# MatteoWohlrapp/mri-inr

Hardware: AMD Instinct MI355X
Metric: Mpixels/sec reconstructed (320x320 slice, hidden=256, 5 layers) (higher is better)
Workload: dtype f16x3

## Files before the change

mri_inr_amd/csrc/diagnostics.hip:

```cpp
#include <algorithm>
#include <vector>

#include "host_ctx.h"
#include "mfma_probe.hip.h"
#include "siren_trunk_f16x3n.hip.h"
#include "siren_trunk_f16x3w.hip.h"
#include "siren_trunk_f32.hip.h"
#include "trunk_instances.h"
#include "launch_dispatch.h"

namespace msiren {
MSIREN_F32_INSTANCES(MSIREN_EXTERN_TRUNK)
MSIREN_F16X3N_INSTANCES(MSIREN_EXTERN_TRUNK)
MSIREN_F16X3W_INSTANCES(MSIREN_EXTERN_TRUNK)
}

using namespace mh;

extern "C" {

int msiren_trunk_timeline(msiren_handle h, const float* mods_dev, int64_t B, float* out_dev, uint64_t* stamps_host) {
    int rc = check(h);
    if (rc) return rc;
    if (h->HP != 256 || h->cfg.activation != MSIREN_ACT_SINE || h->cfg.residual || h->H != 256)
// ... 4 lines not shown
    DevBuf st;
    if ((rc = ensure(h, st, (size_t)grid * 32 * sizeof(uint64_t)))) return rc;
    HIPCHK(hipMemsetAsync(st.p, 0, (size_t)grid * 32 * sizeof(uint64_t), h->sc[h->cur].s));
    msiren::TrunkParams p = make_trunk_params(h, Call{}, mods_dev, h->H, B, out_dev);
    p.stamps = (unsigned long long*)st.p;
    hipLaunchKernelGGL((msiren::siren_trunk_f32_kernel<256, 0, 0, 1>), dim3(grid), dim3(256), 256 * 256 + 256 * 16, h->sc[h->cur].s, p);
    HIPCHK(hipGetLastError());
    HIPCHK(hipMemcpyAsync(stamps_host, st.p, (size_t)grid * 32 * sizeof(uint64_t), hipMemcpyDeviceToHost, h->sc[h->cur].s));
    HIPCHK(hipStreamSynchronize(h->sc[h->cur].s));
    HIPCHK(hipFree(st.p));
    return 0;
}

int msiren_f16x3_timeline(msiren_handle h, const float* mods_dev, int64_t B, float* out_dev, uint64_t* stamps_host) {
    int rc = check(h);
    if (rc) return rc;
    if (!h->f16x3_ready || h->cfg.activation != MSIREN_ACT_SINE) return fail(MSIREN_E_INVALID, "f16x3 timeline: H=256 sine model required");
    msiren::TrunkF16Params p{};
    p.grid = h->d_grid; p.l0 = h->d_l0; p.s0t = h->d_s0t; p.wp = (const _Float16*)h->d_wp16n; p.bias = h->d_bias16;
    p.wout = h->d_wout16; p.mods = mods_dev; p.out = out_dev;
    for (int i = 0; i < 16; ++i) p.winv[i] = h->mscale16[i];
    p.bout = h->bout; p.cg0 = h->cg0; p.cg = h->cg; p.B = (int)B; p.P = h->P; p.L = h->L;
    p.units_per_patch = (h->P + 31) / 32;
    p.total_units = (int)(B * p.units_per_patch);
    const int grid = (int)std::min<int64_t>(h->num_cus, (p.total_units + 3) / 4);
    DevBuf st, q;
    if ((rc = ensure(h, st, (size_t)grid * 4 * 48 * sizeof(uint64_t))) || (rc = ensure(h, q, 256))) return rc;
    hipStream_t s = h->sc[h->cur].s;
    HIPCHK(hipMemsetAsync(st.p, 0, (size_t)grid * 4 * 48 * sizeof(uint64_t), s));
    p.pass_counter = (int*)q.p;
    HIPCHK(hipMemsetAsync(p.pass_counter, 0, 4, s));
    p.pass_base = 0;
    p.stamps = (unsigned long long*)st.p;
    const int lds = msiren::F16Lds<4>::total(h->L);
    {
        if (h->L != 5) return fail(MSIREN_E_INVALID, "f16x3 timeline: the stamped build is the num_layers = 5 instance");
        auto k = msiren::siren_trunk_f16x3n_kernel<0, 4, 5, 1>;
        HIPCHK(hipFuncSetAttribute((const void*)k, hipFuncAttributeMaxDynamicSharedMemorySize, lds));
        hipLaunchKernelGGL(k, dim3(grid), dim3(256), lds, s, p);
    }
    HIPCHK(hipGetLastError());
    HIPCHK(hipMemcpyAsync(stamps_host, st.p, (size_t)grid * 4 * 48 * sizeof(uint64_t), hipMemcpyDeviceToHost, s));
    HIPCHK(hipStreamSynchronize(s));
    HIPCHK(hipFree(st.p));
    HIPCHK(hipFree(q.p));
    return 0;
}

int msiren_f16x3w_timeline(msiren_handle h, const float* mods_dev, int64_t B, float* out_dev, uint64_t* stamps_host) {
    int rc = check(h);
    if (rc) return rc;
    if (!h->f16x3_ready || h->cfg.activation != MSIREN_ACT_SINE || h->L < msiren::WS_MIN_L || h->L > msiren::WS_MAX_L)
        return fail(MSIREN_E_INVALID, "f16x3w timeline: H=256 sine model with %d <= num_layers <= %d required", msiren::WS_MIN_L, msiren::WS_MAX_L);
    if (B <= 0 || !mods_dev || !out_dev || !stamps_host) return fail(MSIREN_E_INVALID, "bad arguments");
    msiren::TrunkWsParams p{};
    if (!h->d_dump) HIPCHK(hipMalloc((void**)&h->d_dump, 256 * sizeof(float)));
    p.dump = h->d_dump;
    p.s0t = h->d_s0t; p.wp = (const _Float16*)h->d_wp16n; p.bias = h->d_bias16; p.wout = h->d_wout16; p.mods = mods_dev; p.out = out_dev;
    for (int i = 0; i < 16; ++i) p.mscale[i] = h->mscale16[i];
    p.bout = h->bout; p.cg0 = h->cg0; p.cg = h->cg; p.B = (int)B; p.P = h->P; p.L = h->L;
    const int upp = (h->P + 31) / 32;
    p.units_per_patch = upp;
    p.total_units = (int)(B * upp);
    int lg = 0;
    while ((1 << lg) < upp) ++lg;
    p.div_k = 30 + lg;
// ... 68 lines not shown
```

mri_inr_amd/csrc/encoder_modulator_f16x3.hip.h:

```cpp
#pragma once
#include <hip/hip_runtime.h>

#include <type_traits>

#include "encoder_params.h"
#include "host_plan.h"

namespace msiren {

typedef _Float16 em_h8 __attribute__((ext_vector_type(8)));
typedef _Float16 em_h2 __attribute__((ext_vector_type(2)));
typedef float em_f4 __attribute__((ext_vector_type(4)));
typedef unsigned em_u4 __attribute__((ext_vector_type(4)));

constexpr int EM_ROWS = 16;
constexpr int EM_C3_KSTEPS = 64;
constexpr int EM_MAX_DEPTH = 16;
constexpr int EM_FC_KSTEPS = 4;

struct EmTailParams {
    const em_u4* wstream;
    const float* bias;
    const em_u4* feat;
    const float* feat_inv;
// ... 456 lines not shown
            for (int t = 0; t < 2; ++t) {
                const int pos = 16 * (2 * (wv >> 1) + t) + n, y = pos >> 3, x = pos & 7;
                const em_u4* src = a1img + ((2 * y + ky) * 17 + 2 * x + kx) * 4 + (q & 1);
                const em_u4 bh = src[0], bl = src[2];
                acc[t] = em_mfma(wa[s][1], bh, acc[t]);
                acc[t] = em_mfma(wa[s][0], bl, acc[t]);
                acc[t] = em_mfma(wa[s][0], bh, acc[t]);
            }
        }
        const float u = inv1 * p.c2_winv;
#pragma unroll
        for (int r = 0; r < 4; ++r) {
            o0[r] = leaky02(__builtin_fmaf(acc[0][r], u, b2[r]));
            o1[r] = leaky02(__builtin_fmaf(acc[1][r], u, b2[r]));
        }
    }
    float m = em_absmax8(o0, o1);
#pragma unroll
    for (int d = 1; d < 64; d <<= 1) m = __builtin_fmaxf(m, __shfl_xor(m, d));
    if (lane == 0) wmax[4 + wv] = m;
    __syncthreads();
    m = __builtin_fmaxf(__builtin_fmaxf(wmax[4], wmax[5]), __builtin_fmaxf(wmax[6], wmax[7]));
    float sc, inv;
    em_row_scale(m, sc, inv);
    em_u4 hi, lo;
    em_split8(o0 * sc, o1 * sc, hi, lo);
    const int row = blockIdx.x, ks = 16 * wv + (lane >> 2), qq = lane & 3;
    em_u4* dst = feat + ((size_t)(row >> 4) * EM_C3_KSTEPS + ks) * 128 + qq * 16 + (row & 15);
    dst[0] = hi;
    dst[64] = lo;
    if (tid == 0) feat_inv[row] = inv;
}

}
```

mri_inr_amd/csrc/host_ctx.h:

```cpp
#pragma once
#include <hip/hip_runtime.h>

#include <cstdint>
#include <map>
#include <string>
#include <vector>

#include "../../include/msiren.h"
#include "dispatch.h"
#include "encoder_params.h"
#include "pass_queue.h"

typedef struct ncclComm* ncclComm_t;

namespace mh {

int fail(int code, const char* fmt, ...) __attribute__((format(printf, 2, 3)));
const char* last_error();

#define HIPCHK(expr)                                                                              \
    do {                                                                                          \
        hipError_t e_ = (expr);                                                                   \
        if (e_ != hipSuccess)                                                                     \
            return ::mh::fail(MSIREN_E_HIP, "%s failed: %s (%s:%d)", #expr, hipGetErrorString(e_), __FILE__, __LINE__); \
    } while (0)

struct DevBuf {
    void* p = nullptr;
    size_t cap = 0;
};

}

struct msiren_ctx {
    msiren_config cfg{};
    int H = 0, HP = 0, L = 0, Z = 0, S = 0, P = 0, O = 0, I = 0;
    struct StreamCtx {
        hipStream_t s = nullptr;
        mh::DevBuf mods, modpad, latent, patches, keep, rec, queue, feat, plan;
        mh::DevBuf score;
        mh::DevBuf cscratch;
        mh::DevBuf coords, l0tab;
        mh::DevBuf ragged;
        struct Lattice {
            int out_stride = 0, tile = 0, pad = 0;
            float *coords = nullptr, *table = nullptr, *foldw = nullptr;
            std::vector<float> host;
        };
        std::vector<Lattice> lattices;
        hipEvent_t ev_join = nullptr;
        msiren::PassQueue pq;
    } sc[3];
    int cur = 0, nstreams = 1;
    msiren::DispatchHandle dh;
    const char* last_trunk = "";
    const char* last_prologue = "";
    struct { const void* k = nullptr; int bytes = 0; } lds_set[8];
    hipEvent_t ev0 = nullptr, ev1 = nullptr;
    std::map<std::string, std::vector<float>> tensors;
    std::map<std::string, size_t> expected;
    std::vector<float> grid_host;
    bool committed = false, have_modulator = false, have_encoder = false;
    float *d_grid = nullptr, *d_l0 = nullptr, *d_wp = nullptr, *d_bias = nullptr, *d_wout = nullptr;
    float *d_w0raw = nullptr, *d_b0raw = nullptr;
    float bout = 0.f, cg0 = 0.f, cg = 0.f;
    void* d_wp16n = nullptr;
    volatile int* status_host = nullptr;
    int* status_dev = nullptr;
    unsigned range_epoch = 0;
    int64_t range_events = 0;
    float* d_dump = nullptr;
    int trace_host = 0;
    float *d_bias16 = nullptr, *d_wout16 = nullptr, *d_s0t = nullptr;
// ... 167 lines not shown
```

mri_inr_amd/csrc/launch_dispatch.h:

```cpp
#pragma once
#include "host_ctx.h"

namespace mh {
msiren::TrunkParams make_trunk_params(msiren_ctx* h, const Call& c, const float* mods, int stride, int64_t B, float* out_dev);
}
```

mri_inr_amd/csrc/launch_dispatch.hip:

```cpp
#include <algorithm>
#include <cstdio>

#include "host_ctx.h"
#include "encoder_modulator.hip.h"
#include "encoder_modulator_f16x3.hip.h"
#include "siren_trunk_f16x3n.hip.h"
#include "siren_trunk_f16x3n_ragged.hip.h"
#include "siren_trunk_f16x3h.hip.h"
#include "siren_trunk_f16x3w.hip.h"
#include "siren_trunk_f32.hip.h"
#include "siren_trunk_f32_jet.hip.h"
#include "siren_trunk_f32_ragged.hip.h"
#include "siren_trunk_x1n.hip.h"
#include "siren_trunk_x1w.hip.h"
#include "tiling.hip.h"
#include "launch_dispatch.h"

namespace msiren {
MSIREN_TRUNK_INSTANCES(MSIREN_EXTERN_TRUNK)
MSIREN_F32_JET_INSTANCES(MSIREN_EXTERN_TRUNK)
MSIREN_F32_RAGGED_INSTANCES(MSIREN_EXTERN_TRUNK)
MSIREN_F32_JET_RAGGED_INSTANCES(MSIREN_EXTERN_TRUNK)
MSIREN_F16X3N_RAGGED_INSTANCES(MSIREN_EXTERN_TRUNK)
MSIREN_F32_RAGGED_COND_INSTANCES(MSIREN_EXTERN_TRUNK)
// ... 183 lines not shown
    p.bias = h->d_bias16;
    p.wout = h->d_wout16;
    p.mods = mods_dev;
    p.out = out_dev;
    for (int i = 0; i < 16; ++i) p.mscale[i] = h->mscale16[i];
    p.bout = h->bout;
    p.cg0 = h->cg0;
    p.cg = h->cg;
    p.B = (int)B;
    p.P = c.P(h);
    p.L = h->L;
    p.plan = c.plan;
    const int upp = (p.P + 31) / 32;
    const int64_t units = B * upp;
    if (units > 0x3fffffffLL) return fail(MSIREN_E_INVALID, "batch too large for one launch: B=%lld", (long long)B);
    p.units_per_patch = upp;
    p.unit_base = 0;
    p.total_units = (int)units;
    {
        int lg = 0;
        while ((1 << lg) < upp) ++lg;
        p.div_k = 30 + lg;
        p.div_m = (unsigned)(((1ULL << p.div_k) + (unsigned)upp - 1) / (unsigned)upp);
    }
    const int grid = (int)std::min<int64_t>(h->num_cus, (units + 1) / 2);
    const msiren::WsSchedule sch = msiren::ws_schedule(units, grid);
    int rc = queue_for_launch(h, c.stream, sch.npasses(), &p.pass_counter, &p.pass_base);
    if (rc) return rc;
    p.status = guard_word(h, t, p.pass_counter);
    p.status_val = (int)h->range_epoch;
    return queue_launched(h, c.stream, launch(h, c.stream, t.inst, grid, msiren::WsLds<4>::total(h->L), p, true));
}

static int launch_trunk_f16x3n(msiren_ctx* h, const Call& c, const msiren::TrunkPick& t, const float* mods_dev, int64_t B, float* out_dev) {
    msiren::TrunkF16Params p{};
    p.grid = c.cs.Q ? c.cs.coords : h->d_grid;
    p.l0 = h->d_l0;
    p.s0t = c.cs.Q ? c.cs.table : h->d_s0t;
    p.wp = (const _Float16*)h->d_wp16n;
    p.bias = h->d_bias16;
    p.wout = h->d_wout16;
    p.mods = mods_dev;
    p.out = out_dev;
    for (int i = 0; i < 16; ++i) p.winv[i] = h->mscale16[i];
    p.bout = h->bout;
    p.cg0 = h->cg0;
    p.cg = h->cg;
    p.B = (int)B;
    p.P = c.P(h);
    p.L = h->L;
    p.plan = c.plan;
    if (B * ((p.P + 31) / 32) > 0x3fffffffLL) return fail(MSIREN_E_INVALID, "batch too large for one launch: B=%lld", (long long)B);
    p.units_per_patch = t.half ? (p.P + 15) / 16 : (p.P + 31) / 32;
    p.unit_base = 0;
    p.total_units = (int)(B * p.units_per_patch);
    const int64_t passes = ((int64_t)p.total_units + 3) / 4;
    const int grid = (int)std::min<int64_t>(h->num_cus, passes);
    int rc = queue_for_launch(h, c.stream, passes, &p.pass_counter, &p.pass_base);
    if (rc) return rc;
    p.status = guard_word(h, t, p.pass_counter);
    p.status_val = (int)h->range_epoch;
    const int lds = t.ring == 4 ? msiren::F16Lds<4>::total(h->L) : msiren::F16Lds<3>::total(h->L);
    return queue_launched(h, c.stream, launch(h, c.stream, t.inst, grid, lds, p, true));
}

static int launch_trunk_x1(msiren_ctx* h, const Call& c, const msiren::TrunkPick& t, const float* mods_dev, int64_t B, float* out_dev) {
    const bool ws = msiren::kInstances[t.inst].family == Kernel::x1w;
    msiren::TrunkX1Params p{};
    p.s0t = c.cs.Q ? c.cs.table : h->d_s0t512;
    p.wp = (const unsigned short*)(ws ? h->d_wpx1w : h->d_wpx1n);
    p.bias32 = h->d_bias32x1;
    p.wout = (const _Float16*)h->d_woutx1;
    p.mods = mods_dev;
    p.out = out_dev;
    for (int i = 0; i < 64; ++i) p.winv[i] = h->winvx1[i];
    p.bout = h->bout;
    p.cg0 = h->cg0;
    p.cg = h->cg;
    p.B = (int)B;
    p.P = c.P(h);
    p.L = h->L;
    p.units_per_patch = (p.P + 31) / 32;
    const int64_t units = B * p.units_per_patch;
    if (units > 0x7fffffffLL) return fail(MSIREN_E_INVALID, "batch too large for one launch: B=%lld", (long long)B);
    p.total_units = (int)units;
    p.plan = c.plan;
    const int grid = t.balanced ? msiren::x1w_balanced_grid(units, h->num_cus) : (int)std::min<int64_t>(h->num_cus, (units + 3) / 4);
    int64_t npasses = (units + 3) / 4;
    if (ws) {
        const msiren::X1wSchedule sch = msiren::x1w_schedule(units, grid);
        npasses = (int64_t)sch.n4 + sch.n2;
    }
    int rc = queue_for_launch(h, c.stream, npasses, &p.pass_counter, &p.pass_base);
    if (rc) return rc;
// ... 627 lines not shown
```

mri_inr_amd/csrc/msiren.hip:

```cpp
#include <dlfcn.h>

#include <chrono>
#include <cstdarg>
#include <cstdio>
#include <cstdlib>
#include <cstring>

#include "host_ctx.h"
#include "host_buffers.h"
#include "host_plan.h"
#include "weights_blob.h"

namespace mh {

namespace {
thread_local std::string g_err;
}

int fail(int code, const char* fmt, ...) {
    char buf[1024];
    va_list ap;
    va_start(ap, fmt);
    vsnprintf(buf, sizeof buf, fmt, ap);
    va_end(ap);
// ... 167 lines not shown
        for (int i = 0; i < 16; ++i) h->status_host[i] = 0;
        e = hipHostGetDevicePointer((void**)&h->status_dev, (void*)h->status_host, 0);
    }

    if (e == hipSuccess) e = hipEventCreate(&h->ev0);
    if (e == hipSuccess) e = hipEventCreate(&h->ev1);
    if (e != hipSuccess) {
        msiren_destroy(h);
        return fail(MSIREN_E_HIP, "context creation failed: %s", hipGetErrorString(e));
    }
    *out = h;
    return 0;
}

int msiren_destroy(msiren_handle h) {
    if (!h) return 0;
    (void)hipSetDevice(h->cfg.device);
    for (auto& c : h->sc)
        if (c.s) (void)hipStreamSynchronize(c.s);
    if (h->comm) (void)comm_destroy(h);
    drop_lattices(h);
    if (h->status_host) (void)hipHostFree((void*)h->status_host);
    if (h->ws_comm.p) (void)hipFree(h->ws_comm.p);
    if (h->d_wp16n) (void)hipFree(h->d_wp16n);
    if (h->d_emw) (void)hipFree(h->d_emw);
    if (h->d_emc2) (void)hipFree(h->d_emc2);
    for (void* q : {h->d_woutx1, h->d_wpx1n, h->d_wpx1w, (void*)h->d_bias32x1})
        if (q) (void)hipFree(q);
    float* ptrs[] = {h->d_w0raw, h->d_b0raw, h->d_dump, h->d_s0t512, h->d_s0t, h->d_bias16, h->d_wout16, h->d_grid, h->d_l0, h->d_wp, h->d_bias, h->d_wout, h->d_modw, h->d_modw_rm, h->d_modb, h->d_encw, h->d_foldw, h->d_embias};
    for (float* p : ptrs)
        if (p) (void)hipFree(p);
    std::vector<DevBuf*> bufs = {&h->stage_in, &h->stage_out};
    for (auto& c : h->sc)
        for (DevBuf* b : {&c.cscratch, &c.mods, &c.modpad, &c.latent, &c.patches, &c.keep, &c.rec, &c.queue, &c.feat, &c.plan, &c.score, &c.coords, &c.l0tab, &c.ragged}) bufs.push_back(b);
    for (DevBuf* b : bufs)
        if (b->p) (void)hipFree(b->p);
    for (auto& pr : h->prof_events) {
        (void)hipEventDestroy(pr.a);
        (void)hipEventDestroy(pr.b);
    }
    for (auto& c : h->sc)
        if (c.ev_join) (void)hipEventDestroy(c.ev_join);
    if (h->ev0) (void)hipEventDestroy(h->ev0);
    if (h->ev1) (void)hipEventDestroy(h->ev1);
    for (auto& c : h->sc)
        if (c.s) (void)hipStreamDestroy(c.s);
    delete h;
    return 0;
}

int msiren_set_tensor(msiren_handle h, const char* name, const float* host_data, size_t n) {
    if (!h || !name || (!host_data && n)) return fail(MSIREN_E_INVALID, "null argument");
    auto it = h->expected.find(name);
    if (it == h->expected.end()) return fail(MSIREN_E_INVALID, "Unexpected key in state_dict: \"%s\"", name);
    if (it->second != n)
        return fail(MSIREN_E_SHAPE, "size mismatch for %s: got %zu elements, the configuration implies %zu", name, n, it->second);
    h->tensors[name].assign(host_data, host_data + n);
    h->committed = false;
    return 0;
}

int msiren_get_tensor(msiren_handle h, const char* name, float* host_out, size_t n) {
    if (!h || !name || (!host_out && n)) return fail(MSIREN_E_INVALID, "null argument");
    auto ex = h->expected.find(name);
    if (ex == h->expected.end()) return fail(MSIREN_E_INVALID, "Unexpected key in state_dict: \"%s\"", name);
    auto it = h->tensors.find(name);
    if (it == h->tensors.end()) return fail(MSIREN_E_STATE, "tensor %s has not been set", name);
// ... 505 lines not shown
```

mri_inr_amd/csrc/siren_trunk_f16x3h.hip.h:

```cpp
#pragma once
#include <hip/hip_runtime.h>

#include "siren_trunk_f16x3n.hip.h"

namespace msiren {

template <int ACT, int R, int LFIX = 0>
__global__ __launch_bounds__(256, 1) void siren_trunk_f16x3h_kernel(TrunkF16Params p) {
    using LY = F16Lds<R>;
    extern __shared__ __attribute__((aligned(16))) unsigned char smem[];
    const int tid = threadIdx.x;
    const int lane = tid & 63;
    const int wave = __builtin_amdgcn_readfirstlane(tid >> 6);
    const int q = lane >> 4;
    const int n16 = lane & 15;
    const int L = p.L;
    const int nchunks = (L - 1) * 8;

    const unsigned char* woutB = smem + LY::wout + q * 16;
    const unsigned char* zeroB = smem + LY::zero + q * 16;
    const unsigned char* biasB = smem + LY::bias + q * 16;
    float* modT = reinterpret_cast<float*>(smem + LY::mods(L)) + wave * (L * 256);
    const unsigned char* modB = reinterpret_cast<const unsigned char*>(modT) + q * 16;

    {
        f32x4* l0w = reinterpret_cast<f32x4*>(smem + LY::l0);
        float* wow = reinterpret_cast<float*>(smem + LY::wout);
        float* zw = reinterpret_cast<float*>(smem + LY::zero);
        float* bw = reinterpret_cast<float*>(smem + LY::bias);
        l0w[tid] = reinterpret_cast<const f32x4*>(p.l0)[tid];
        wow[tid] = p.wout[tid];
        zw[tid] = 0.f;
        for (int i = tid; i < (L - 1) * 256; i += 256) bw[i] = p.bias[i];
    }

    volatile int* qslot = reinterpret_cast<volatile int*>(smem + LY::queue(L));
    float* mscaleT = reinterpret_cast<float*>(smem + LY::winv(L));
    if (tid < 16) mscaleT[tid] = p.winv[tid];
    int cur_pass = (int)blockIdx.x;
    const unsigned char* wsrc = reinterpret_cast<const unsigned char*>(p.wp) + wave * 8192 + lane * 16 + 4096;
    int dma_id = 0, dma_buf = 0, rd_buf = 0;
    const unsigned char* dsrc_ = wsrc;
    unsigned char* ddst_ = smem + LY::ring + wave * 8192 + 4096;
    auto dma_begin = [&]() {
        dsrc_ = wsrc + (size_t)dma_id * F16_CHUNK_BYTES;
        ddst_ = smem + LY::ring + dma_buf * F16_CHUNK_BYTES + wave * 8192 + 4096;
        dma_id = dma_id + 1 == nchunks ? 0 : dma_id + 1;
        dma_buf = dma_buf + 1 == R ? 0 : dma_buf + 1;
    };
#define MSIREN_DMA_PIECE(I)                                                                               \
    __builtin_amdgcn_global_load_lds((const __attribute__((address_space(1))) void*)dsrc_,                \
                                     (__attribute__((address_space(3))) void*)ddst_, 16, (I) * 1024 - 4096, 0)
    auto dma_next = [&]() {
        dma_begin();
        MSIREN_DMA_PIECE(0);
        MSIREN_DMA_PIECE(1);
        MSIREN_DMA_PIECE(2);
        MSIREN_DMA_PIECE(3);
        MSIREN_DMA_PIECE(4);
        MSIREN_DMA_PIECE(5);
        MSIREN_DMA_PIECE(6);
        MSIREN_DMA_PIECE(7);
    };
    const int total_units = __builtin_amdgcn_readfirstlane(p.plan ? p.plan[1] : p.total_units);
    const unsigned npasses = (unsigned)(total_units + 3) >> 2;
    if ((unsigned)cur_pass >= npasses) return;
#pragma unroll
    for (int s = 0; s < R - 1; ++s) dma_next();

    h8 Xh[8], Xl[8], Yh[8], Yl[8];
    f32x4 acc[2][2];
    float part4[4] = {0.f, 0.f, 0.f, 0.f};

    fp16x2 eh[2][2], el[2][2];
    f32x4 tb_m[2], bia[2];
    auto tbl_load = [&](int sub, const unsigned char* ml, const unsigned char* wo, int t, bool withw) {
        const int fo = (32 * t + 16 * sub) * 4;
        tb_m[sub] = *reinterpret_cast<const f32x4*>(ml + fo);
        if (withw) tb_m[sub] *= *reinterpret_cast<const f32x4*>(wo + fo);
    };
    auto bias_load = [&](int sub, const unsigned char* bl, int t) {
        bia[sub] = *reinterpret_cast<const f32x4*>(bl + (32 * t + 16 * sub) * 4);
        asm("; bias fragment stays in arch VGPRs" : "+v"(bia[sub]));
    };
    auto epi_half = [&](const f32x4& a, float cgl, int sub, int hh, bool lastl, bool fresh = false, int chain = 0, bool ready = false) {
        float v[2];
        if (fresh) {
            v[0] = ready ? a[2 * hh] : activate<ACT>(a[2 * hh], cgl);
            v[1] = ready ? a[2 * hh + 1] : activate<ACT>(a[2 * hh + 1], cgl);
        } else if constexpr (ACT == 0) {
            asm volatile("v_sin_f32 %0, %1" : "=v"(v[0]) : "v"(a[2 * hh]));
            asm volatile("v_sin_f32 %0, %1" : "=v"(v[1]) : "v"(a[2 * hh + 1]));
        } else {
            float s0, s1, t0, t1;
            asm volatile("v_sin_f32 %0, %2\n\tv_mul_f32 %1, %3, %2" : "=&v"(s0), "=&v"(t0) : "v"(a[2 * hh]), "v"(cgl));
            asm volatile("v_sin_f32 %0, %2\n\tv_mul_f32 %1, %3, %2" : "=&v"(s1), "=&v"(t1) : "v"(a[2 * hh + 1]), "v"(cgl));
            v[0] = s0 * __builtin_amdgcn_exp2f(t0 * a[2 * hh]);
            v[1] = s1 * __builtin_amdgcn_exp2f(t1 * a[2 * hh + 1]);
        }
// ... 81 lines not shown
        const unsigned char* mlp_ = modB + (l_ - 1) * 1024;                                   \
        MSIREN_H16_TILE(INh, INl, OUTh, OUTl, 0, LASTF);                                        \
        MSIREN_H16_TILE(INh, INl, OUTh, OUTl, 1, LASTF);                                        \
        MSIREN_H16_TILE(INh, INl, OUTh, OUTl, 2, LASTF);                                        \
        MSIREN_H16_TILE(INh, INl, OUTh, OUTl, 3, LASTF);                                        \
        MSIREN_H16_TILE(INh, INl, OUTh, OUTl, 4, LASTF);                                        \
        MSIREN_H16_TILE(INh, INl, OUTh, OUTl, 5, LASTF);                                        \
        MSIREN_H16_TILE(INh, INl, OUTh, OUTl, 6, LASTF);                                        \
        MSIREN_H16_TILE(INh, INl, OUTh, OUTl, 7, LASTF);                                        \
    } while (0)

    asm volatile("s_waitcnt vmcnt(%0)" ::"n"((R - 2) * 8) : "memory");
    __syncthreads();
    bias_load(0, biasB, 0);
    bias_load(1, biasB, 0);
    {
        const h8* r0 = reinterpret_cast<const h8*>(smem + LY::ring) + lane;
        wf_[0][0] = r0[0 * 64];
        wf_[0][1] = r0[1 * 64];
        wf_[0][2] = r0[2 * 64];
        wf_[0][3] = r0[3 * 64];
    }

    for (int pass = 0; (unsigned)cur_pass < npasses; ++pass) {
        int unit = cur_pass * 4 + wave;
        const bool active = unit < total_units;
        unit = (active ? unit : total_units - 1) + p.unit_base;
        const int b = unit / p.units_per_patch;
        const int cu = unit - b * p.units_per_patch;
        int pc0 = cu * 16 + n16;
        const bool pv0 = active && pc0 < p.P;
        pc0 = pc0 < p.P ? pc0 : p.P - 1;

        int nxt = 0;
        if (tid == 0) nxt = (int)((unsigned)atomicAdd(p.pass_counter, 1) - p.pass_base) + (int)gridDim.x;
        bool bad_mod = false;
        for (int l = 0; l < L; ++l) {
            const f32x4 m = *reinterpret_cast<const f32x4*>(p.mods + ((size_t)l * p.B + b) * 256 + lane * 4);
            const f32x4 ms = m * mscaleT[l];
            bad_mod |= f16_out_of_range(ms);
            *reinterpret_cast<f32x4*>(modT + l * 256 + lane * 4) = ms;
        }
        if (bad_mod && p.status) *p.status = p.status_val;
        if (tid == 0) qslot[(pass + 1) & 1] = nxt;

        const f32x4* s0a = reinterpret_cast<const f32x4*>(p.s0t) + (size_t)q * p.P + pc0;
        f32x4 raw[7][2];
#pragma unroll
        for (int s = 0; s < 7; ++s)
#pragma unroll
            for (int sub = 0; sub < 2; ++sub) raw[s][sub] = s0a[(size_t)(8 * s + 4 * sub) * p.P];
#pragma unroll
        for (int s = 0; s < 7; ++s) {
            fp16x2 hh[2][2], ll[2][2];
#pragma unroll
            for (int sub = 0; sub < 2; ++sub) {
                const f32x4 m4 = *reinterpret_cast<const f32x4*>(modB + (32 * s + 16 * sub) * 4);
                const f32x4 a = raw[s][sub];
                split_products_pk(a[0], m4[0], a[1], m4[1], hh[sub][0], ll[sub][0]);
                split_products_pk(a[2], m4[2], a[3], m4[3], hh[sub][1], ll[sub][1]);
            }
            Xh[s] = to_acc_file(pack_h8(hh[0][0], hh[0][1], hh[1][0], hh[1][1]));
            Xl[s] = to_acc_file(pack_h8(ll[0][0], ll[0][1], ll[1][0], ll[1][1]));
        }
#pragma unroll
        for (int sub = 0; sub < 2; ++sub) acc[1][sub] = s0a[(size_t)(56 + 4 * sub) * p.P];
        tbl_load(0, modB, zeroB, 7, false);

        part4[0] = part4[1] = part4[2] = part4[3] = 0.f;
        if constexpr (LFIX == 5) {
            MSIREN_H16_LAYER(Xh, Xl, Yh, Yl, 1, false);
            MSIREN_H16_LAYER(Yh, Yl, Xh, Xl, 2, false);
            MSIREN_H16_LAYER(Xh, Xl, Yh, Yl, 3, false);
            MSIREN_H16_LAYER(Yh, Yl, Xh, Xl, 4, true);
        } else {
            for (int l = 1;;) {
                if (l == L - 1) {
                    MSIREN_H16_LAYER(Xh, Xl, Yh, Yl, l, true);
                    break;
                }
                MSIREN_H16_LAYER(Xh, Xl, Yh, Yl, l, false);
                ++l;
                if (l == L - 1) {
                    MSIREN_H16_LAYER(Yh, Yl, Xh, Xl, l, true);
                    break;
                }
                MSIREN_H16_LAYER(Yh, Yl, Xh, Xl, l, false);
                ++l;
            }
        }
        tbl_load(1, modB + (L - 1) * 1024, woutB, 7, true);
#pragma unroll
        for (int sub = 0; sub < 2; ++sub) {
            epi_half(acc[1][sub], p.cg, sub, 0, true, true, 3);
            epi_half(acc[1][sub], p.cg, sub, 1, true, true, 3);
        }
        const float sv = (sum_over_q(part4[0]) + sum_over_q(part4[1])) + (sum_over_q(part4[2]) + sum_over_q(part4[3]));
        if (q == 0 && pv0) p.out[(size_t)b * p.P + pc0] = sin_rev(sv + p.bout);
        cur_pass = __builtin_amdgcn_readfirstlane(qslot[(pass + 1) & 1]);
// ... 11 lines not shown
```

mri_inr_amd/csrc/siren_trunk_f16x3n.hip.h:

```cpp
#pragma once
#include <hip/hip_runtime.h>

#include "siren_trunk_f16_common.hip.h"

namespace msiren {

__device__ __forceinline__ void mfma_n16_first(f32x4& d, const h8& a, const h8& b, const f32x4& c) {
    d = __builtin_amdgcn_mfma_f32_16x16x32_f16(a, b, c, 0, 0, 0);
}
__device__ __forceinline__ void mfma_n16_acc(f32x4& d, const h8& a, const h8& b) {
    d = __builtin_amdgcn_mfma_f32_16x16x32_f16(a, b, d, 0, 0, 0);
}

__device__ __forceinline__ void split_products_pk(float a0, float m0, float a1, float m1, fp16x2& hi, fp16x2& lo) {
    unsigned h, l;
    asm("v_fma_mixlo_f16 %0, %1, %2, 0 op_sel_hi:[0,0,0]" : "=v"(h) : "v"(a0), "v"(m0));
    asm("v_fma_mixhi_f16 %0, %1, %2, 0 op_sel_hi:[0,0,0]" : "+v"(h) : "v"(a1), "v"(m1));
    asm("v_fma_mixlo_f16 %0, %1, %2, -%3 op_sel:[0,0,0] op_sel_hi:[0,0,1]" : "=v"(l) : "v"(a0), "v"(m0), "v"(h));
    asm("v_fma_mixhi_f16 %0, %1, %2, -%3 op_sel:[0,0,1] op_sel_hi:[0,0,1]" : "+v"(l) : "v"(a1), "v"(m1), "v"(h));
    hi = __builtin_bit_cast(fp16x2, h);
    lo = __builtin_bit_cast(fp16x2, l);
}

__device__ __forceinline__ float sum_over_q(float x) {
    float a = x, b = x;
    asm volatile("s_nop 1\n\tv_permlane16_swap_b32 %0, %1" : "+v"(a), "+v"(b));
    a += b;
    b = a;
    asm volatile("s_nop 1\n\tv_permlane32_swap_b32 %0, %1" : "+v"(a), "+v"(b));
    return a + b;
}


template <int ACT, int R, int LFIX = 0, int DBG = 0>
__global__ __launch_bounds__(256, 1) void siren_trunk_f16x3n_kernel(TrunkF16Params p) {
    using LY = F16Lds<R>;
    extern __shared__ __attribute__((aligned(16))) unsigned char smem[];
    const int tid = threadIdx.x;
    const int lane = tid & 63;
    const int wave = __builtin_amdgcn_readfirstlane(tid >> 6);
    const int q = lane >> 4;
    const int n16 = lane & 15;
    const int L = p.L;
    const int nchunks = (L - 1) * 8;

    const unsigned char* woutB = smem + LY::wout + q * 16;
    const unsigned char* zeroB = smem + LY::zero + q * 16;
    const unsigned char* biasB = smem + LY::bias + q * 16;
    float* modT = reinterpret_cast<float*>(smem + LY::mods(L)) + wave * (L * 256);
    const unsigned char* modB = reinterpret_cast<const unsigned char*>(modT) + q * 16;

    {
        f32x4* l0w = reinterpret_cast<f32x4*>(smem + LY::l0);
        float* wow = reinterpret_cast<float*>(smem + LY::wout);
        float* zw = reinterpret_cast<float*>(smem + LY::zero);
        float* bw = reinterpret_cast<float*>(smem + LY::bias);
        l0w[tid] = reinterpret_cast<const f32x4*>(p.l0)[tid];
        wow[tid] = p.wout[tid];
        zw[tid] = 0.f;
        for (int i = tid; i < (L - 1) * 256; i += 256) bw[i] = p.bias[i];
    }

    volatile int* qslot = reinterpret_cast<volatile int*>(smem + LY::queue(L));
    float* mscaleT = reinterpret_cast<float*>(smem + LY::winv(L));
    if (tid < 16) mscaleT[tid] = p.winv[tid];
    int cur_pass = (int)blockIdx.x;
    const unsigned char* wsrc = reinterpret_cast<const unsigned char*>(p.wp) + wave * 8192 + lane * 16 + 4096;
    int dma_id = 0, dma_buf = 0, rd_buf = 0;
    const unsigned char* dsrc_ = wsrc;
    unsigned char* ddst_ = smem + LY::ring + wave * 8192 + 4096;
    auto dma_begin = [&]() {
        dsrc_ = wsrc + (size_t)dma_id * F16_CHUNK_BYTES;
        ddst_ = smem + LY::ring + dma_buf * F16_CHUNK_BYTES + wave * 8192 + 4096;
        dma_id = dma_id + 1 == nchunks ? 0 : dma_id + 1;
        dma_buf = dma_buf + 1 == R ? 0 : dma_buf + 1;
    };
#define MSIREN_DMA_PIECE(I)                                                                               \
    __builtin_amdgcn_global_load_lds((const __attribute__((address_space(1))) void*)dsrc_,                \
                                     (__attribute__((address_space(3))) void*)ddst_, 16, (I) * 1024 - 4096, 0)
    auto dma_next = [&]() {
        dma_begin();
        MSIREN_DMA_PIECE(0);
        MSIREN_DMA_PIECE(1);
        MSIREN_DMA_PIECE(2);
        MSIREN_DMA_PIECE(3);
        MSIREN_DMA_PIECE(4);
        MSIREN_DMA_PIECE(5);
        MSIREN_DMA_PIECE(6);
        MSIREN_DMA_PIECE(7);
    };
    const int total_units = __builtin_amdgcn_readfirstlane(p.plan ? p.plan[1] : p.total_units);
    const unsigned npasses = (unsigned)(total_units + 3) >> 2;
    if ((unsigned)cur_pass >= npasses) return;
#pragma unroll
    for (int s = 0; s < R - 1; ++s) dma_next();

    h8 Xh[16], Xl[16], Yh[16], Yl[16];
    f32x4 acc[2][4];
    float part4[2][4] = {{0.f, 0.f, 0.f, 0.f}, {0.f, 0.f, 0.f, 0.f}};

    fp16x2 eh[4][2], el[4][2];
    f32x4 tb_m[2], bia[2];
    auto tbl_load = [&](int sub, const unsigned char* ml, const unsigned char* wo, int t, bool withw) {
        const int fo = (32 * t + 16 * sub) * 4;
        tb_m[sub] = *reinterpret_cast<const f32x4*>(ml + fo);
        if (withw) tb_m[sub] *= *reinterpret_cast<const f32x4*>(wo + fo);
    };
    auto bias_load = [&](int sub, const unsigned char* bl, int t) {
        bia[sub] = *reinterpret_cast<const f32x4*>(bl + (32 * t + 16 * sub) * 4);
        asm("; bias fragment stays in arch VGPRs" : "+v"(bia[sub]));
    };
    auto epi_half = [&](const f32x4& a, float cgl, int pt, int hh, bool lastl, bool fresh = false, int chain = 0, bool ready = false) {
        const int sub = pt & 1, g = pt >> 1;
        float v[2];
        if (fresh) {
            v[0] = ready ? a[2 * hh] : activate<ACT>(a[2 * hh], cgl);
            v[1] = ready ? a[2 * hh + 1] : activate<ACT>(a[2 * hh + 1], cgl);
        } else if constexpr (ACT == 0) {
            asm volatile("v_sin_f32 %0, %1" : "=v"(v[0]) : "v"(a[2 * hh]));
            asm volatile("v_sin_f32 %0, %1" : "=v"(v[1]) : "v"(a[2 * hh + 1]));
        } else {
            float s0, s1, t0, t1;
            asm volatile("v_sin_f32 %0, %2\n\tv_mul_f32 %1, %3, %2" : "=&v"(s0), "=&v"(t0) : "v"(a[2 * hh]), "v"(cgl));
            asm volatile("v_sin_f32 %0, %2\n\tv_mul_f32 %1, %3, %2" : "=&v"(s1), "=&v"(t1) : "v"(a[2 * hh + 1]), "v"(cgl));
            v[0] = s0 * __builtin_amdgcn_exp2f(t0 * a[2 * hh]);
            v[1] = s1 * __builtin_amdgcn_exp2f(t1 * a[2 * hh + 1]);
// ... 231 lines not shown

    asm volatile("s_waitcnt vmcnt(%0)" ::"n"((R - 2) * 8) : "memory");
    __syncthreads();
    bias_load(0, biasB, 0);
    bias_load(1, biasB, 0);
    {
        const h8* r0 = reinterpret_cast<const h8*>(smem + LY::ring) + lane;
        wf_[0][0] = r0[0 * 64];
        wf_[0][1] = r0[1 * 64];
        wf_[0][2] = r0[2 * 64];
        wf_[0][3] = r0[3 * 64];
    }

    for (int pass = 0; (unsigned)cur_pass < npasses; ++pass) {
        auto stamp = [&](int i) {
            if constexpr (DBG) {
                const unsigned long long t = i == 7 ? __builtin_amdgcn_s_memrealtime() : __builtin_amdgcn_s_memtime();
                if (tid == 0 && pass < 4) p.stamps[((size_t)blockIdx.x * 4 + pass) * 48 + i] = t;
            }
        };
        stamp(0);
        int dbg_tile = 0;
        (void)dbg_tile;
        int unit = cur_pass * 4 + wave;
        const bool active = unit < total_units;
        unit = (active ? unit : total_units - 1) + p.unit_base;
        const int b = unit / p.units_per_patch;
        const int cu = unit - b * p.units_per_patch;
        int pc0 = cu * 32 + n16, pc1 = cu * 32 + 16 + n16;
        const bool pv0 = active && pc0 < p.P, pv1 = active && pc1 < p.P;
        pc0 = pc0 < p.P ? pc0 : p.P - 1;
        pc1 = pc1 < p.P ? pc1 : p.P - 1;

        int nxt = 0;
        if (tid == 0) nxt = (int)((unsigned)atomicAdd(p.pass_counter, 1) - p.pass_base) + (int)gridDim.x;
        bool bad_mod = false;
        for (int l = 0; l < L; ++l) {
            const f32x4 m = *reinterpret_cast<const f32x4*>(p.mods + ((size_t)l * p.B + b) * 256 + lane * 4);
            const f32x4 ms = m * mscaleT[l];
            bad_mod |= f16_out_of_range(ms);
            *reinterpret_cast<f32x4*>(modT + l * 256 + lane * 4) = ms;
        }
        if (bad_mod && p.status) *p.status = p.status_val;
        if (tid == 0) qslot[(pass + 1) & 1] = nxt;

        const f32x4* s0a = reinterpret_cast<const f32x4*>(p.s0t) + (size_t)q * p.P + pc0;
        const f32x4* s0b = reinterpret_cast<const f32x4*>(p.s0t) + (size_t)q * p.P + pc1;
        f32x4 raw[14][2];
#pragma unroll
        for (int s = 0; s < 7; ++s)
#pragma unroll
            for (int sub = 0; sub < 2; ++sub) {
                raw[2 * s + 0][sub] = s0a[(size_t)(8 * s + 4 * sub) * p.P];
                raw[2 * s + 1][sub] = s0b[(size_t)(8 * s + 4 * sub) * p.P];
            }
#pragma unroll
        for (int s = 0; s < 7; ++s) {
            f32x4 m4[2];
#pragma unroll
            for (int sub = 0; sub < 2; ++sub) m4[sub] = *reinterpret_cast<const f32x4*>(modB + (32 * s + 16 * sub) * 4);
#pragma unroll
            for (int g = 0; g < 2; ++g) {
                fp16x2 hh[2][2], ll[2][2];
#pragma unroll
                for (int sub = 0; sub < 2; ++sub) {
                    const f32x4 a = raw[2 * s + g][sub];
                    split_products_pk(a[0], m4[sub][0], a[1], m4[sub][1], hh[sub][0], ll[sub][0]);
                    split_products_pk(a[2], m4[sub][2], a[3], m4[sub][3], hh[sub][1], ll[sub][1]);
                }
                Xh[2 * s + g] = to_acc_file(pack_h8(hh[0][0], hh[0][1], hh[1][0], hh[1][1]));
                Xl[2 * s + g] = to_acc_file(pack_h8(ll[0][0], ll[0][1], ll[1][0], ll[1][1]));
            }
        }
#pragma unroll
        for (int sub = 0; sub < 2; ++sub) {
            acc[1][0 + sub] = s0a[(size_t)(56 + 4 * sub) * p.P];
            acc[1][2 + sub] = s0b[(size_t)(56 + 4 * sub) * p.P];
        }
        tbl_load(0, modB, zeroB, 7, false);

#pragma unroll
        for (int c = 0; c < 4; ++c) part4[0][c] = part4[1][c] = 0.f;
        stamp(1);
        if constexpr (LFIX == 5) {
            MSIREN_N16_LAYER(Xh, Xl, Yh, Yl, 1, false);
            MSIREN_N16_LAYER(Yh, Yl, Xh, Xl, 2, false);
            MSIREN_N16_LAYER(Xh, Xl, Yh, Yl, 3, false);
            MSIREN_N16_LAYER(Yh, Yl, Xh, Xl, 4, true);
        } else {
            for (int l = 1;;) {
                if (l == L - 1) {
                    MSIREN_N16_LAYER(Xh, Xl, Yh, Yl, l, true);
                    break;
                }
                MSIREN_N16_LAYER(Xh, Xl, Yh, Yl, l, false);
                ++l;
                if (l == L - 1) {
                    MSIREN_N16_LAYER(Yh, Yl, Xh, Xl, l, true);
                    break;
                }
                MSIREN_N16_LAYER(Yh, Yl, Xh, Xl, l, false);
                ++l;
            }
        }
        stamp(2);
        tbl_load(1, modB + (L - 1) * 1024, woutB, 7, true);
#pragma unroll
        for (int pt = 0; pt < 4; ++pt) {
            epi_half(acc[1][pt], p.cg, pt, 0, true, true, 3);
            epi_half(acc[1][pt], p.cg, pt, 1, true, true, 3);
        }
// ... 23 lines not shown
```

Before: 385.9.

## Prescale modulations in a staging kernel and DMA them directly into LDS

Adds a small pre-pass kernel that multiplies the modulations by their per-layer f16 scale and checks their range once per batch row. For the L=5 f16x3n path, and unconditionally in the f16x3h kernel, the trunk then streams mods, l0, bias and wout into LDS with global_load_lds_dwordx4 instead of loading through registers, scaling and storing them. The s0 tail loads move earlier behind an explicit waitcnt, and the pass-counter atomic result is published later to overlap its latency. This removes per-pass VALU work and register round-trips, at the cost of an extra kernel launch plus a round trip of the mods through a global staging buffer.

```diff
diff --git a/mri_inr_amd/csrc/diagnostics.hip b/mri_inr_amd/csrc/diagnostics.hip
--- a/mri_inr_amd/csrc/diagnostics.hip
+++ b/mri_inr_amd/csrc/diagnostics.hip
@@ -60,6 +60,7 @@
     HIPCHK(hipMemsetAsync(p.pass_counter, 0, 4, s));
     p.pass_base = 0;
     p.stamps = (unsigned long long*)st.p;
+    if ((rc = stage_mods_f16x3(h, h->cur, mods_dev, B, nullptr, nullptr, 0, &p.mods))) return rc;
     const int lds = msiren::F16Lds<4>::total(h->L);
     {
         if (h->L != 5) return fail(MSIREN_E_INVALID, "f16x3 timeline: the stamped build is the num_layers = 5 instance");
diff --git a/mri_inr_amd/csrc/encoder_modulator_f16x3.hip.h b/mri_inr_amd/csrc/encoder_modulator_f16x3.hip.h
--- a/mri_inr_amd/csrc/encoder_modulator_f16x3.hip.h
+++ b/mri_inr_amd/csrc/encoder_modulator_f16x3.hip.h
@@ -512,4 +512,31 @@
     if (tid == 0) feat_inv[row] = inv;
 }
 
-}
+struct StageModsParams {
+    const float* mods;
+    float* staged;
+    float scale[16];
+    int B, L;
+    const int* count;
+    int* status;
+    int status_val;
+};
+
+template <int ROWS_PER_BLOCK = 4>
+__global__ __launch_bounds__(256) void stage_mods_f16x3_kernel(StageModsParams p) {
+    const int nrows = p.count ? *p.count : p.B;
+    const int64_t row = (int64_t)blockIdx.x * ROWS_PER_BLOCK + (threadIdx.x >> 6);
+    if (row >= nrows) return;
+    const int lane = threadIdx.x & 63;
+    bool bad = false;
+    for (int l = 0; l < p.L; ++l) {
+        const size_t at = ((size_t)l * p.B + row) * 256 + lane * 4;
+        const em_f4 ms = *reinterpret_cast<const em_f4*>(p.mods + at) * p.scale[l];
+#pragma unroll
+        for (int r = 0; r < 4; ++r) bad |= !(__builtin_fabsf(ms[r]) <= 65504.f);
+        *reinterpret_cast<em_f4*>(p.staged + at) = ms;
+    }
+    if (bad && p.status) *p.status = p.status_val;
+}
+
+}
diff --git a/mri_inr_amd/csrc/host_ctx.h b/mri_inr_amd/csrc/host_ctx.h
--- a/mri_inr_amd/csrc/host_ctx.h
+++ b/mri_inr_amd/csrc/host_ctx.h
@@ -39,6 +39,7 @@
         hipStream_t s = nullptr;
         mh::DevBuf mods, modpad, latent, patches, keep, rec, queue, feat, plan;
         mh::DevBuf score;
+        mh::DevBuf smods;
         mh::DevBuf cscratch;
         mh::DevBuf coords, l0tab;
         mh::DevBuf ragged;
diff --git a/mri_inr_amd/csrc/launch_dispatch.h b/mri_inr_amd/csrc/launch_dispatch.h
--- a/mri_inr_amd/csrc/launch_dispatch.h
+++ b/mri_inr_amd/csrc/launch_dispatch.h
@@ -3,4 +3,5 @@
 
 namespace mh {
 msiren::TrunkParams make_trunk_params(msiren_ctx* h, const Call& c, const float* mods, int stride, int64_t B, float* out_dev);
+int stage_mods_f16x3(msiren_ctx* h, int s, const float* mods_dev, int64_t B, const int* count, int* status, int status_val, const float** staged);
 }
diff --git a/mri_inr_amd/csrc/launch_dispatch.hip b/mri_inr_amd/csrc/launch_dispatch.hip
--- a/mri_inr_amd/csrc/launch_dispatch.hip
+++ b/mri_inr_amd/csrc/launch_dispatch.hip
@@ -239,6 +239,25 @@
     return queue_launched(h, c.stream, launch(h, c.stream, t.inst, grid, msiren::WsLds<4>::total(h->L), p, true));
 }
 
+int stage_mods_f16x3(msiren_ctx* h, int s, const float* mods_dev, int64_t B, const int* count, int* status, int status_val, const float** staged) {
+    auto& sc = h->sc[s];
+    int rc = ensure(h, sc.smods, (size_t)h->L * B * 256 * sizeof(float));
+    if (rc) return rc;
+    msiren::StageModsParams sp{};
+    sp.mods = mods_dev;
+    sp.staged = (float*)sc.smods.p;
+    for (int i = 0; i < 16; ++i) sp.scale[i] = h->mscale16[i];
+    sp.B = (int)B;
+    sp.L = h->L;
+    sp.count = count;
+    sp.status = status;
+    sp.status_val = status_val;
+    hipLaunchKernelGGL(msiren::stage_mods_f16x3_kernel<4>, dim3((unsigned)((B + 3) / 4)), dim3(256), 0, sc.s, sp);
+    HIPCHK(hipGetLastError());
+    *staged = sp.staged;
+    return 0;
+}
+
 static int launch_trunk_f16x3n(msiren_ctx* h, const Call& c, const msiren::TrunkPick& t, const float* mods_dev, int64_t B, float* out_dev) {
     msiren::TrunkF16Params p{};
     p.grid = c.cs.Q ? c.cs.coords : h->d_grid;
@@ -267,6 +286,7 @@
     if (rc) return rc;
     p.status = guard_word(h, t, p.pass_counter);
     p.status_val = (int)h->range_epoch;
+    if (h->L == 5 && (rc = stage_mods_f16x3(h, c.stream, mods_dev, B, c.plan, p.status, p.status_val, &p.mods))) return queue_launched(h, c.stream, rc);
     const int lds = t.ring == 4 ? msiren::F16Lds<4>::total(h->L) : msiren::F16Lds<3>::total(h->L);
     return queue_launched(h, c.stream, launch(h, c.stream, t.inst, grid, lds, p, true));
 }
diff --git a/mri_inr_amd/csrc/msiren.hip b/mri_inr_amd/csrc/msiren.hip
--- a/mri_inr_amd/csrc/msiren.hip
+++ b/mri_inr_amd/csrc/msiren.hip
@@ -223,7 +223,7 @@
         if (p) (void)hipFree(p);
     std::vector<DevBuf*> bufs = {&h->stage_in, &h->stage_out};
     for (auto& c : h->sc)
-        for (DevBuf* b : {&c.cscratch, &c.mods, &c.modpad, &c.latent, &c.patches, &c.keep, &c.rec, &c.queue, &c.feat, &c.plan, &c.score, &c.coords, &c.l0tab, &c.ragged}) bufs.push_back(b);
+        for (DevBuf* b : {&c.cscratch, &c.smods, &c.mods, &c.modpad, &c.latent, &c.patches, &c.keep, &c.rec, &c.queue, &c.feat, &c.plan, &c.score, &c.coords, &c.l0tab, &c.ragged}) bufs.push_back(b);
     for (DevBuf* b : bufs)
         if (b->p) (void)hipFree(b->p);
     for (auto& pr : h->prof_events) {
diff --git a/mri_inr_amd/csrc/siren_trunk_f16x3h.hip.h b/mri_inr_amd/csrc/siren_trunk_f16x3h.hip.h
--- a/mri_inr_amd/csrc/siren_trunk_f16x3h.hip.h
+++ b/mri_inr_amd/csrc/siren_trunk_f16x3h.hip.h
@@ -23,20 +23,7 @@
     float* modT = reinterpret_cast<float*>(smem + LY::mods(L)) + wave * (L * 256);
     const unsigned char* modB = reinterpret_cast<const unsigned char*>(modT) + q * 16;
 
-    {
-        f32x4* l0w = reinterpret_cast<f32x4*>(smem + LY::l0);
-        float* wow = reinterpret_cast<float*>(smem + LY::wout);
-        float* zw = reinterpret_cast<float*>(smem + LY::zero);
-        float* bw = reinterpret_cast<float*>(smem + LY::bias);
-        l0w[tid] = reinterpret_cast<const f32x4*>(p.l0)[tid];
-        wow[tid] = p.wout[tid];
-        zw[tid] = 0.f;
-        for (int i = tid; i < (L - 1) * 256; i += 256) bw[i] = p.bias[i];
-    }
-
-    volatile int* qslot = reinterpret_cast<volatile int*>(smem + LY::queue(L));
-    float* mscaleT = reinterpret_cast<float*>(smem + LY::winv(L));
-    if (tid < 16) mscaleT[tid] = p.winv[tid];
+    volatile __attribute__((address_space(3))) int* qslot = (volatile __attribute__((address_space(3))) int*)(smem + LY::queue(L));
     int cur_pass = (int)blockIdx.x;
     const unsigned char* wsrc = reinterpret_cast<const unsigned char*>(p.wp) + wave * 8192 + lane * 16 + 4096;
     int dma_id = 0, dma_buf = 0, rd_buf = 0;
@@ -65,6 +52,13 @@
     const int total_units = __builtin_amdgcn_readfirstlane(p.plan ? p.plan[1] : p.total_units);
     const unsigned npasses = (unsigned)(total_units + 3) >> 2;
     if ((unsigned)cur_pass >= npasses) return;
+    {
+        copy_1kb_to_lds(reinterpret_cast<const unsigned char*>(p.l0) + wave * 1024 + lane * 16, lds_address(smem + LY::l0) + wave * 1024);
+        for (int l = wave; l < L - 1; l += 4)
+            copy_1kb_to_lds(reinterpret_cast<const unsigned char*>(p.bias) + l * 1024 + lane * 16, lds_address(smem + LY::bias) + l * 1024);
+        if (wave == 0) copy_1kb_to_lds(reinterpret_cast<const unsigned char*>(p.wout) + lane * 16, lds_address(smem + LY::wout));
+        reinterpret_cast<float*>(smem + LY::zero)[tid] = 0.f;
+    }
 #pragma unroll
     for (int s = 0; s < R - 1; ++s) dma_next();
 
@@ -212,17 +206,19 @@
         const bool pv0 = active && pc0 < p.P;
         pc0 = pc0 < p.P ? pc0 : p.P - 1;
 
-        int nxt = 0;
-        if (tid == 0) nxt = (int)((unsigned)atomicAdd(p.pass_counter, 1) - p.pass_base) + (int)gridDim.x;
-        bool bad_mod = false;
-        for (int l = 0; l < L; ++l) {
-            const f32x4 m = *reinterpret_cast<const f32x4*>(p.mods + ((size_t)l * p.B + b) * 256 + lane * 4);
-            const f32x4 ms = m * mscaleT[l];
-            bad_mod |= f16_out_of_range(ms);
-            *reinterpret_cast<f32x4*>(modT + l * 256 + lane * 4) = ms;
-        }
-        if (bad_mod && p.status) *p.status = p.status_val;
-        if (tid == 0) qslot[(pass + 1) & 1] = nxt;
+        unsigned got = 0;
+        if (tid == 0) {
+            __attribute__((address_space(1))) int* pc = (__attribute__((address_space(1))) int*)p.pass_counter;
+            asm("" : "+v"(pc));
+            got = (unsigned)__hip_atomic_fetch_add(pc, 1, __ATOMIC_RELAXED, __HIP_MEMORY_SCOPE_AGENT);
+        }
+        {
+            const unsigned char* msrc = reinterpret_cast<const unsigned char*>(p.mods + (size_t)b * 256) + lane * 16;
+            const size_t mstep = (size_t)p.B * 1024;
+            const unsigned mdst = lds_address(modT);
+            for (int l = 0; l < L; ++l) copy_1kb_to_lds(msrc + l * mstep, mdst + l * 1024);
+        }
+        __builtin_amdgcn_sched_barrier(0);
 
         const f32x4* s0a = reinterpret_cast<const f32x4*>(p.s0t) + (size_t)q * p.P + pc0;
         f32x4 raw[7][2];
@@ -230,6 +226,10 @@
         for (int s = 0; s < 7; ++s)
 #pragma unroll
             for (int sub = 0; sub < 2; ++sub) raw[s][sub] = s0a[(size_t)(8 * s + 4 * sub) * p.P];
+#pragma unroll
+        for (int sub = 0; sub < 2; ++sub) acc[1][sub] = s0a[(size_t)(56 + 4 * sub) * p.P];
+        asm volatile("" ::: "memory");
+        __builtin_amdgcn_s_waitcnt(0x4F70);
 #pragma unroll
         for (int s = 0; s < 7; ++s) {
             fp16x2 hh[2][2], ll[2][2];
@@ -243,8 +243,7 @@
             Xh[s] = to_acc_file(pack_h8(hh[0][0], hh[0][1], hh[1][0], hh[1][1]));
             Xl[s] = to_acc_file(pack_h8(ll[0][0], ll[0][1], ll[1][0], ll[1][1]));
         }
-#pragma unroll
-        for (int sub = 0; sub < 2; ++sub) acc[1][sub] = s0a[(size_t)(56 + 4 * sub) * p.P];
+        if (tid == 0) qslot[(pass + 1) & 1] = (int)(got - p.pass_base) + (int)gridDim.x;
         tbl_load(0, modB, zeroB, 7, false);
 
         part4[0] = part4[1] = part4[2] = part4[3] = 0.f;
diff --git a/mri_inr_amd/csrc/siren_trunk_f16x3n.hip.h b/mri_inr_amd/csrc/siren_trunk_f16x3n.hip.h
--- a/mri_inr_amd/csrc/siren_trunk_f16x3n.hip.h
+++ b/mri_inr_amd/csrc/siren_trunk_f16x3n.hip.h
@@ -30,6 +30,11 @@
     asm volatile("s_nop 1\n\tv_permlane32_swap_b32 %0, %1" : "+v"(a), "+v"(b));
     return a + b;
 }
+
+__device__ __forceinline__ void copy_1kb_to_lds(const void* src, unsigned lds) {
+    asm volatile("s_mov_b32 m0, %1\n\ts_nop 0\n\tglobal_load_lds_dwordx4 %0, off" ::"v"(src), "s"(lds) : "memory", "m0");
+}
+__device__ __forceinline__ unsigned lds_address(const void* p) { return (unsigned)(size_t)(const __attribute__((address_space(3))) void*)p; }
 
 
 template <int ACT, int R, int LFIX = 0, int DBG = 0>
@@ -43,6 +48,9 @@
     const int n16 = lane & 15;
     const int L = p.L;
     const int nchunks = (L - 1) * 8;
+    if constexpr (DBG) {
+        if (tid == 0) p.stamps[(size_t)blockIdx.x * 4 * 48 + 3] = __builtin_amdgcn_s_memtime();
+    }
 
     const unsigned char* woutB = smem + LY::wout + q * 16;
     const unsigned char* zeroB = smem + LY::zero + q * 16;
@@ -50,20 +58,7 @@
     float* modT = reinterpret_cast<float*>(smem + LY::mods(L)) + wave * (L * 256);
     const unsigned char* modB = reinterpret_cast<const unsigned char*>(modT) + q * 16;
 
-    {
-        f32x4* l0w = reinterpret_cast<f32x4*>(smem + LY::l0);
-        float* wow = reinterpret_cast<float*>(smem + LY::wout);
-        float* zw = reinterpret_cast<float*>(smem + LY::zero);
-        float* bw = reinterpret_cast<float*>(smem + LY::bias);
-        l0w[tid] = reinterpret_cast<const f32x4*>(p.l0)[tid];
-        wow[tid] = p.wout[tid];
-        zw[tid] = 0.f;
-        for (int i = tid; i < (L - 1) * 256; i += 256) bw[i] = p.bias[i];
-    }
-
-    volatile int* qslot = reinterpret_cast<volatile int*>(smem + LY::queue(L));
-    float* mscaleT = reinterpret_cast<float*>(smem + LY::winv(L));
-    if (tid < 16) mscaleT[tid] = p.winv[tid];
+    volatile __attribute__((address_space(3))) int* qslot = (volatile __attribute__((address_space(3))) int*)(smem + LY::queue(L));
     int cur_pass = (int)blockIdx.x;
     const unsigned char* wsrc = reinterpret_cast<const unsigned char*>(p.wp) + wave * 8192 + lane * 16 + 4096;
     int dma_id = 0, dma_buf = 0, rd_buf = 0;
@@ -92,6 +87,23 @@
     const int total_units = __builtin_amdgcn_readfirstlane(p.plan ? p.plan[1] : p.total_units);
     const unsigned npasses = (unsigned)(total_units + 3) >> 2;
     if ((unsigned)cur_pass >= npasses) return;
+    if constexpr (LFIX != 0) {
+        copy_1kb_to_lds(reinterpret_cast<const unsigned char*>(p.l0) + wave * 1024 + lane * 16, lds_address(smem + LY::l0) + wave * 1024);
+        for (int l = wave; l < L - 1; l += 4)
+            copy_1kb_to_lds(reinterpret_cast<const unsigned char*>(p.bias) + l * 1024 + lane * 16, lds_address(smem + LY::bias) + l * 1024);
+        if (wave == 0) copy_1kb_to_lds(reinterpret_cast<const unsigned char*>(p.wout) + lane * 16, lds_address(smem + LY::wout));
+        reinterpret_cast<float*>(smem + LY::zero)[tid] = 0.f;
+    } else {
+        f32x4* l0w = reinterpret_cast<f32x4*>(smem + LY::l0);
+        float* wow = reinterpret_cast<float*>(smem + LY::wout);
+        float* zw = reinterpret_cast<float*>(smem + LY::zero);
+        float* bw = reinterpret_cast<float*>(smem + LY::bias);
+        l0w[tid] = reinterpret_cast<const f32x4*>(p.l0)[tid];
+        wow[tid] = p.wout[tid];
+        zw[tid] = 0.f;
+        for (int i = tid; i < (L - 1) * 256; i += 256) bw[i] = p.bias[i];
+        if (tid < 16) reinterpret_cast<float*>(smem + LY::winv(L))[tid] = p.winv[tid];
+    }
 #pragma unroll
     for (int s = 0; s < R - 1; ++s) dma_next();
 
@@ -389,21 +401,33 @@
         pc0 = pc0 < p.P ? pc0 : p.P - 1;
         pc1 = pc1 < p.P ? pc1 : p.P - 1;
 
-        int nxt = 0;
-        if (tid == 0) nxt = (int)((unsigned)atomicAdd(p.pass_counter, 1) - p.pass_base) + (int)gridDim.x;
-        bool bad_mod = false;
-        for (int l = 0; l < L; ++l) {
-            const f32x4 m = *reinterpret_cast<const f32x4*>(p.mods + ((size_t)l * p.B + b) * 256 + lane * 4);
-            const f32x4 ms = m * mscaleT[l];
-            bad_mod |= f16_out_of_range(ms);
-            *reinterpret_cast<f32x4*>(modT + l * 256 + lane * 4) = ms;
-        }
-        if (bad_mod && p.status) *p.status = p.status_val;
-        if (tid == 0) qslot[(pass + 1) & 1] = nxt;
+        unsigned got = 0;
+        if (tid == 0) {
+            __attribute__((address_space(1))) int* pc = (__attribute__((address_space(1))) int*)p.pass_counter;
+            asm("" : "+v"(pc));
+            got = (unsigned)__hip_atomic_fetch_add(pc, 1, __ATOMIC_RELAXED, __HIP_MEMORY_SCOPE_AGENT);
+        }
+        if constexpr (LFIX != 0) {
+            const unsigned char* msrc = reinterpret_cast<const unsigned char*>(p.mods + (size_t)b * 256) + lane * 16;
+            const size_t mstep = (size_t)p.B * 1024;
+            const unsigned mdst = lds_address(modT);
+            for (int l = 0; l < L; ++l) copy_1kb_to_lds(msrc + l * mstep, mdst + l * 1024);
+        } else {
+            const float* mscaleT = reinterpret_cast<const float*>(smem + LY::winv(L));
+            bool bad_mod = false;
+            for (int l = 0; l < L; ++l) {
+                const f32x4 m = *reinterpret_cast<const f32x4*>(p.mods + ((size_t)l * p.B + b) * 256 + lane * 4);
+                const f32x4 ms = m * mscaleT[l];
+                bad_mod |= f16_out_of_range(ms);
+                *reinterpret_cast<f32x4*>(modT + l * 256 + lane * 4) = ms;
+            }
+            if (bad_mod && p.status) *p.status = p.status_val;
+        }
 
         const f32x4* s0a = reinterpret_cast<const f32x4*>(p.s0t) + (size_t)q * p.P + pc0;
         const f32x4* s0b = reinterpret_cast<const f32x4*>(p.s0t) + (size_t)q * p.P + pc1;
         f32x4 raw[14][2];
+        if constexpr (LFIX != 0) __builtin_amdgcn_sched_barrier(0);
 #pragma unroll
         for (int s = 0; s < 7; ++s)
 #pragma unroll
@@ -411,6 +435,15 @@
                 raw[2 * s + 0][sub] = s0a[(size_t)(8 * s + 4 * sub) * p.P];
                 raw[2 * s + 1][sub] = s0b[(size_t)(8 * s + 4 * sub) * p.P];
             }
+        if constexpr (LFIX != 0) {
+#pragma unroll
+            for (int sub = 0; sub < 2; ++sub) {
+                acc[1][0 + sub] = s0a[(size_t)(56 + 4 * sub) * p.P];
+                acc[1][2 + sub] = s0b[(size_t)(56 + 4 * sub) * p.P];
+            }
+            asm volatile("" ::: "memory");
+            __builtin_amdgcn_s_waitcnt(0x8F70);
+        }
 #pragma unroll
         for (int s = 0; s < 7; ++s) {
             f32x4 m4[2];
@@ -429,11 +462,14 @@
                 Xl[2 * s + g] = to_acc_file(pack_h8(ll[0][0], ll[0][1], ll[1][0], ll[1][1]));
             }
         }
-#pragma unroll
-        for (int sub = 0; sub < 2; ++sub) {
-            acc[1][0 + sub] = s0a[(size_t)(56 + 4 * sub) * p.P];
-            acc[1][2 + sub] = s0b[(size_t)(56 + 4 * sub) * p.P];
-        }
+        if constexpr (LFIX == 0) {
+#pragma unroll
+            for (int sub = 0; sub < 2; ++sub) {
+                acc[1][0 + sub] = s0a[(size_t)(56 + 4 * sub) * p.P];
+                acc[1][2 + sub] = s0b[(size_t)(56 + 4 * sub) * p.P];
+            }
+        }
+        if (tid == 0) qslot[(pass + 1) & 1] = (int)(got - p.pass_base) + (int)gridDim.x;
         tbl_load(0, modB, zeroB, 7, false);
 
 #pragma unroll
```

Result: no change. 389.3, median of 6 (+0.9%).
